# Zeng-Yan/centermask2

Measured on AMD Instinct MI355X. Metric: images/sec whole-node (V2-39-eSE 3x800x1280), higher is better.
Workload: dtype f32

## Files before the change

centermask2_amd/csrc/conv_args.hpp:

```cpp
#pragma once
#include "cmk_common.hpp"

namespace cmk {

typedef float f32x16 __attribute__((ext_vector_type(16)));
typedef float f32x4 __attribute__((ext_vector_type(4)));

constexpr int PST = 20;
constexpr int MAXP = 10;
constexpr int LDS_CU = 160 * 1024;

__host__ __device__ constexpr int occ_of(int wm, int wn, int stride) { return (stride == 1 && (wm == 1 ? wn <= 5 : wn <= 2)) ? 3 : 2; }

struct ConvProblem {
    const float* x; float* y; const float* scale; const float* shift;
    const float* in_scale; const float* in_shift;
    const float* w;
    float acc_scale;
    int N, H, W, Ho, Wo;
    int tiles_h, tiles_w, tile_begin;
    long total_pix;
};

struct ConvArgs {
// ... 7 lines not shown
    int total_tiles;
    int ksplit;
    float* ws;
    double* gn_ws;
    int gn_cpg, gn_groups;
    int ga_stride;
    float* pool_ws;
    int grid_y;
};

struct DeviceOnce {
    unsigned char done[64] = {0};
    template <typename F>
    int run(F&& f) {
        int dev = 0;
        if (hipGetDevice(&dev) != hipSuccess || dev < 0 || dev >= 64) return fail(CMK_ELAUNCH, "hipGetDevice failed%s", "");
        if (__atomic_load_n(&done[dev], __ATOMIC_ACQUIRE)) return CMK_OK;
        int rc = f();
        if (rc == CMK_OK) __atomic_store_n(&done[dev], 1, __ATOMIC_RELEASE);
        return rc;
    }
};

int launch_wino6(ConvArgs& a, int geo, hipStream_t st);
int launch_wino6s(ConvArgs& a, int geo, hipStream_t st);
int launch_pw(ConvArgs& a, int mt, hipStream_t st);
int launch_pw_split(ConvArgs& a, int mode, hipStream_t st);
int launch_sp3(ConvArgs& a, int geo, int pieces, hipStream_t st);

}
```

centermask2_amd/csrc/conv_igemm.hip:

```cpp
#include <stdlib.h>

#include "conv_args.hpp"

namespace cmk {

template <int TAPS, int STRIDE, int WM, int WN, int SC>
struct Geo {
    static constexpr int SR = 32 / SC;
    static constexpr int SUBT = 4 * WM;
    static constexpr int BM = 32 * SUBT;
    static constexpr int BN = 32 * WN;
    static constexpr int TH = (TAPS == 9) ? SR * SUBT : 1;
    static constexpr int TW = (TAPS == 9) ? SC : BM;
    static constexpr int HH = (TAPS == 9) ? (TH - 1) * STRIDE + 3 : 1;
    static constexpr int HWD = (TAPS == 9) ? (TW - 1) * STRIDE + 3 : BM;
    static constexpr int APIX = HH * HWD;
    static constexpr int A_BYTES = APIX * PST * 4;
    static constexpr int B_BYTES = BN * PST * 4;
    static constexpr int OCC = occ_of(WM, WN, STRIDE);
    static constexpr bool ADB = (2 * A_BYTES + 2 * B_BYTES) * OCC <= LDS_CU;
    static constexpr int LDS_BYTES = (ADB ? 2 : 1) * A_BYTES + 2 * B_BYTES;
    static constexpr int RESIDENT = (LDS_BYTES * OCC <= LDS_CU) ? OCC : (LDS_BYTES * 2 <= LDS_CU ? 2 : 1);
    static constexpr int A_ITERS = (APIX * 4 + 255) / 256;
    static constexpr int B_ITERS = (BN * 4 + 255) / 256;
// ... 853 lines not shown

static int dispatch(ConvArgs& a, const cmk_conv_desc* d, const cmk_conv_desc* descs, int n, hipStream_t st) {
    const int cout32 = (d->Cout + 31) / 32;
    if (d->gn_ws) {
        if (d->tune_wm != 5 && d->tune_wm != 6 && d->tune_wm != 11)
            return fail(CMK_EINVAL, "conv: fused GroupNorm statistics are only produced by the Winograd form%s", "");
        int rc = setup_gn(a, d);
        if (rc) return rc;
    }
    if (d->tune_wm == 5) {
        if (d->ksize != 3 || d->stride != 1 || d->res_mode != 0 || d->in_relu || !d->w_wino)
            return fail(CMK_EINVAL, "conv: Winograd variant not available for this conv%s", "");
        if (d->splitk > 1) return fail(CMK_EINVAL, "conv: split-K is a direct-kernel feature%s", "");
        a.w = d->w_wino;
        return launch_wino(a, st);
    }
    if (d->tune_wm == 6) {
        if (d->ksize != 3 || d->stride != 1 || d->res_mode != 0 || d->in_relu || !d->w_wino6 || (d->Cin & 7))
            return fail(CMK_EINVAL, "conv: Winograd F(4x4,3x3) variant not available for this conv%s", "");
        a.w = d->w_wino6;
        a.ws = d->splitk_ws;
        a.ksplit = d->splitk > 1 ? d->splitk : 1;
        a.cout_pad = cmk_conv_cout_pad(d->Cout);
        if (a.ksplit > 1) {
            if (d->tune_sc == 64 || d->tune_wn != 1 || n != 1) return fail(CMK_EINVAL, "conv: Winograd split-K needs tune_sc 16, tune_wn 1, one problem%s", "");
            return launch_wino6(a, 0, st);
        }
        if (d->tune_wn != 1 && d->tune_wn != 2) return fail(CMK_EINVAL, "conv: tune_wm 6 takes tune_wn 1 (12x40 map tiles) or 2 (pairs of RoI maps up to 16x14)%s", "");
        if (d->tune_sc == 64) return launch_wino6s(a, d->tune_wn == 2 ? 1 : 0, st);
        return launch_wino6(a, d->tune_wn == 2 ? 1 : 0, st);
    }
    a.ksplit = d->splitk > 1 ? d->splitk : 1;
    a.ws = d->splitk_ws;
    if (d->pool_ws && !pointwise_mt(d, n)) return fail(CMK_EINVAL, "conv: pooled sums are produced by the pointwise GEMM kernel only (cmk_conv_pool_rows)%s", "");
    a.pool_ws = d->pool_ws;
    if (d->tune_wm == 8) {
        if (d->ksize != 1 || cout32 <= 7) return fail(CMK_EINVAL, "conv: pointwise variant needs a 1x1 conv with Cout > 224%s", "");
        a.cout_pad = cdiv(cout32, 4) * 128;
        if (a.ksplit > 1 && !pointwise_mt(d, n)) return fail(CMK_EINVAL, "conv: pointwise variant: split-K not available for this conv%s", "");
        return launch_pw(a, d->tune_wn, st);
    }
    if (d->tune_wm == 10) {
        if (!(d->ksize == 1 ? pointwise_mt(d, n) : gather_mt(d, n)))
            return fail(CMK_EINVAL, "conv: the bf16-split variant needs w_split and a conv the pointwise GEMM kernel takes (1x1, or 3x3 in its gather form)%s", "");
        a.cout_pad = cdiv(cout32, 4) * 128;
        a.w = reinterpret_cast<const float*>(d->w_split);
        a.ksplit = 1;
        a.ga_stride = d->ksize == 3 ? d->stride : 0;
        return launch_pw_split(a, 1, st);
    }
    if (d->tune_wm == 12) {
        if (!(d->ksize == 1 ? pointwise_mt(d, n) : gather_mt(d, n)) || !(d->w_splith_scale > 0.f))
            return fail(CMK_EINVAL, "conv: the fp16-split variant needs w_splith, w_splith_scale and a conv the pointwise GEMM kernel takes (1x1, or 3x3 in its gather form)%s", "");
// ... 132 lines not shown
```

centermask2_amd/csrc/conv_wino6.hip:

```cpp
#include <type_traits>

#include "wino6_common.hpp"

namespace cmk {

constexpr int W6_EX_FLOATS = 4 * 4 * 2 * 8 * 64;
template <int GEO> constexpr int w6_lds_bytes() { return (2 * W6G<GEO>::WB * 16 > W6_EX_FLOATS * 4) ? 2 * W6G<GEO>::WB * 16 : W6_EX_FLOATS * 4; }
static_assert(2 * w6_lds_bytes<0>() <= LDS_CU && 2 * w6_lds_bytes<1>() <= LDS_CU, "two workgroups per CU");

template <bool AFF, int GEO>
__global__ __launch_bounds__(256, 2) void conv_wino6_kernel(const ConvArgs a) {
    using G = W6G<GEO>;
    constexpr int W6_AP = G::AP, W6_WB = G::WB;
    extern __shared__ __attribute__((aligned(16))) float smem[];
    f32x4* sW = reinterpret_cast<f32x4*>(smem);

    const int tid = threadIdx.x;
    const int lane = tid & 63;
    const int wave = __builtin_amdgcn_readfirstlane(tid >> 6);
    const int hh = lane >> 5, li = lane & 31;

    const int xq = blockIdx.x >> 3, xcd = blockIdx.x & 7;
    const int bx = (xq / a.grid_y) * 8 + xcd, by = xq % a.grid_y;
    if (bx >= a.total_tiles) return;
    int pi = 0;
#pragma unroll
    for (int i = 1; i < MAXP; ++i)
        if (i < a.nprob && bx >= a.p[i].tile_begin) pi = i;
    const ConvProblem& P = a.p[pi];
    const int H = P.H, W = P.W;
    const int tile = bx - P.tile_begin;
    int n, oh0, ow0;
    if (GEO == 0) {
        const int tw = tile % P.tiles_w;
        const int t2 = tile / P.tiles_w;
        const int th = t2 % P.tiles_h;
        n = t2 / P.tiles_h;
        oh0 = th * G::OH; ow0 = tw * G::OW;
    } else {
        n = tile * 2; oh0 = 0; ow0 = 0;
    }
    const int co0 = by * 32;
    const int ks = blockIdx.y;
    const int c_lo = (int)((long)ks * (a.Cin >> 3) / a.ksplit);
    const int nchunks = (int)((long)(ks + 1) * (a.Cin >> 3) / a.ksplit);

    int p_img, p_q, p_t, p_col;
    bool p_active;
    G::item_of(tid, p_img, p_q, p_t, p_col, p_active);
    i32x4 rsrc;
    {
        const int img_n = n + (GEO == 1 ? (wave >> 1) : 0);
        const unsigned long long base = (unsigned long long)(P.x + (long)min(img_n, P.N - 1) * H * W * a.x_cs);
        rsrc.x = __builtin_amdgcn_readfirstlane((int)(base & 0xffffffffull));
        rsrc.y = __builtin_amdgcn_readfirstlane((int)((base >> 32) & 0xffffull));
        rsrc.z = __builtin_amdgcn_readfirstlane(img_n < P.N ? H * W * a.x_cs * 4 : 0);
        rsrc.w = 0x00020000;
    }
    const int row_bytes = W * a.x_cs * 4;
    const int ih0 = oh0 - 1 + 4 * p_t, iw = ow0 - 1 + p_col;
    const int voff0 = (iw >= 0 && iw < W) ? (ih0 * W + iw) * a.x_cs * 4 + (a.x_co + p_q * 4) * 4 : (int)0x80000000;
    unsigned okm = 0;
    if (AFF) {
#pragma unroll
        for (int i = 0; i < 6; ++i) okm |= ((iw >= 0 && iw < W && ih0 + i >= 0 && ih0 + i < H) ? 1u : 0u) << i;
    }
    const unsigned aff_off = AFF ? (unsigned)(min(n + p_img, P.N - 1) * a.Cin + p_q * 4) : 0u;
    const f32x2 five = {5.0f, 5.0f};
    f32x4 d[6];
    f32x4 in_sc = {1.f, 1.f, 1.f, 1.f}, in_sh = {0.f, 0.f, 0.f, 0.f};
    auto load_D = [&](int chunk) {
#pragma unroll
        for (int i = 0; i < 6; ++i) d[i] = w6_buffer_load(rsrc, voff0 + i * row_bytes, chunk * 32, 0);
        if (AFF) {
            in_sc = *reinterpret_cast<const f32x4*>(P.in_scale + chunk * 8 + aff_off);
            in_sh = *reinterpret_cast<const f32x4*>(P.in_shift + chunk * 8 + aff_off);
        }
    };
    const int p_dst = w6_slot<GEO>(p_q, (GEO == 1 ? 4 * p_img : 0) + p_t, 0, p_col);
    auto pass1 = [&](f32x4* wbuf) {
        if (AFF) {
#pragma unroll
            for (int i = 0; i < 6; ++i) {
                const float kinf = ((okm >> i) & 1u) ? __builtin_inff() : 0.f;
                const f32x4 v = __builtin_elementwise_fma(d[i], in_sc, in_sh);
                d[i] = f32x4{__builtin_amdgcn_fmed3f(v.x, 0.f, kinf), __builtin_amdgcn_fmed3f(v.y, 0.f, kinf),
                             __builtin_amdgcn_fmed3f(v.z, 0.f, kinf), __builtin_amdgcn_fmed3f(v.w, 0.f, kinf)};
            }
        }
        f32x2* dst = reinterpret_cast<f32x2*>(wbuf + p_dst);
        if (GEO == 1 && !p_active) return;
#pragma unroll
        for (int h = 0; h < 2; ++h) {
            f32x2 e[6];
#pragma unroll
            for (int i = 0; i < 6; ++i) e[i] = h ? f32x2{d[i].z, d[i].w} : f32x2{d[i].x, d[i].y};
            f32x2 w0, w1, w2, w3, w4, w5;
            w6_half_first(e[0], e[1], e[2], e[3], e[4], five, w0, w1, w2);
            w6_half_second(e[1], e[2], e[3], e[4], e[5], five, w3, w4, w5);
            dst[0 * 2 * W6_AP + h] = w0; dst[1 * 2 * W6_AP + h] = w1; dst[2 * 2 * W6_AP + h] = w2;
            dst[3 * 2 * W6_AP + h] = w3; dst[4 * 2 * W6_AP + h] = w4; dst[5 * 2 * W6_AP + h] = w5;
        }
    };

    const int rowA = wave, rowB = 4 + (wave >> 1), halfB = wave & 1;
    int m_img, m_t, m_tc;
    G::tile_of(min(li, G::TILES - 1), m_img, m_t, m_tc);
    const f32x4* wl = sW + w6_slot<GEO>(hh, (GEO == 1 ? 4 * m_img : 0) + m_t, 0, 4 * m_tc);
    const f32x4* wA = wl + rowA * W6_AP;
    const f32x4* wB = wl + rowB * W6_AP;
    const f32x4* wBa = wB + (halfB ? G::CK : 0);
    const f32x4* wB3 = wB + (halfB ? 1 : 3 * G::CK);
    const float* u_wave = P.w + ((long)by * 4 + wave) * (9 * 256);
    const long u_chunk = (long)a.grid_y * (36 * 256);
    const int u_lane_off = lane * 4;
    f32x4 ub[3][3];
    auto load_U = [&](int step, int buf) {
        const int c = step / 3, s = step - c * 3;
        const float* src = u_wave + c * u_chunk + s * (3 * 256);
#pragma unroll
        for (int k = 0; k < 3; ++k) ub[buf][k] = *reinterpret_cast<const f32x4*>(src + (u_lane_off + k * 256));
    };
    const int total_steps = nchunks * 3;

    if (GEO == 1) {
        for (int i = tid; i < 2 * 2 * G::RG * 6 * 3; i += 256) {
            const int c3 = i % 3, rest = i / 3;
            const int a6 = rest % 6, r2 = rest / 6;
            const int r = r2 % G::RG, qb = r2 / G::RG;
            sW[(qb >> 1) * G::WB + w6_slot<GEO>(qb & 1, r, a6, 15 + c3)] = f32x4{0.f, 0.f, 0.f, 0.f};
        }
    }
    load_D(c_lo);
    f32x4 d_first[6];
#pragma unroll
    for (int i = 0; i < 6; ++i) d_first[i] = d[i];
    f32x4 sc_first = in_sc, sh_first = in_sh;
    load_D(min(c_lo + 1, nchunks - 1));
    load_U(c_lo * 3, 0);
    load_U(min(c_lo * 3 + 1, total_steps - 1), 1);
    {
        f32x4 d_keep[6], sc_keep = in_sc, sh_keep = in_sh;
#pragma unroll
        for (int i = 0; i < 6; ++i) { d_keep[i] = d[i]; d[i] = d_first[i]; }
        in_sc = sc_first; in_sh = sh_first;
        pass1(sW);
#pragma unroll
        for (int i = 0; i < 6; ++i) d[i] = d_keep[i];
        in_sc = sc_keep; in_sh = sh_keep;
    }

    f32x16 acc[9];
#pragma unroll
    for (int f = 0; f < 9; ++f)
#pragma unroll
        for (int r = 0; r < 16; ++r) acc[f][r] = 0.f;

    struct X5 { f32x2 x0, x1, x2, x3, x4; };
    auto rd = [&](const f32x4* wrow, bool second, int h) {
        const f32x2* w2 = reinterpret_cast<const f32x2*>(wrow) + h;
        X5 x;
        constexpr int K = G::CK;
        if (!second) { x.x0 = w2[0 * 2]; x.x1 = w2[K * 2]; x.x2 = w2[2 * K * 2]; x.x3 = w2[3 * K * 2]; x.x4 = w2[1 * 2]; }
        else         { x.x0 = w2[K * 2]; x.x1 = w2[2 * K * 2]; x.x2 = w2[3 * K * 2]; x.x3 = w2[1 * 2]; x.x4 = w2[(K + 1) * 2]; }
        return x;
// ... 10 lines not shown
        for (int s = 0; s < 2; ++s) {
            acc[abase + 0] = __builtin_amdgcn_mfma_f32_32x32x2f32(v0[s], ub[sbuf][0][2 * h + s], acc[abase + 0], 0, 0, 0);
            acc[abase + 1] = __builtin_amdgcn_mfma_f32_32x32x2f32(v1[s], ub[sbuf][1][2 * h + s], acc[abase + 1], 0, 0, 0);
            acc[abase + 2] = __builtin_amdgcn_mfma_f32_32x32x2f32(v2[s], ub[sbuf][2][2 * h + s], acc[abase + 2], 0, 0, 0);
        }
    };
    auto half_step = [&](const X5& x, bool second, int h, int sbuf, int abase) {
        f32x2 v0, v1, v2;
        if (!second) w6_half_first(x.x0, x.x1, x.x2, x.x3, x.x4, five, v0, v1, v2);
        else w6_half_second(x.x0, x.x1, x.x2, x.x3, x.x4, five, v0, v1, v2);
        mm(v0, v1, v2, h, sbuf, abase);
    };
    auto half_stepB = [&](const X5& x, int h) {
        f32x2 v0, v1, v2;
        if (halfB == 0) { asm volatile("" ::: "memory"); w6_half_first(x.x0, x.x1, x.x2, x.x3, x.x4, five, v0, v1, v2); }
        else            { asm volatile("" ::: "memory"); w6_half_second(x.x0, x.x1, x.x2, x.x3, x.x4, five, v0, v1, v2); }
        mm(v0, v1, v2, h, 2, 6);
    };
    auto period = [&](const int c, auto parity) {
        constexpr int wcur = decltype(parity)::value * W6_WB;
        f32x4* wnext = sW + (1 - decltype(parity)::value) * W6_WB;
        const int step = c * 3;
        __syncthreads();
        constexpr bool AHEAD = !AFF;
        load_U(min(step + 2, total_steps - 1), 2);
        X5 xa = rd(wA + wcur, false, 0), xb;
        if (AHEAD) xb = rd(wA + wcur, false, 1);
        half_step(xa, false, 0, 0, 0);
        if (AHEAD) xa = rd(wA + wcur, true, 0); else xb = rd(wA + wcur, false, 1);
        half_step(xb, false, 1, 0, 0);
        __builtin_amdgcn_sched_barrier(0);
        pass1(wnext);
        load_D(min(c + 2, nchunks - 1));
        __builtin_amdgcn_sched_barrier(0);
        load_U(min(step + 3, total_steps - 1), 0);
        if (AHEAD) xb = rd(wA + wcur, true, 1); else xa = rd(wA + wcur, true, 0);
        half_step(xa, true, 0, 1, 3);
        if (AHEAD) xa = rdB(wBa + wcur, wB3 + wcur, 0); else xb = rd(wA + wcur, true, 1);
        half_step(xb, true, 1, 1, 3);
        __builtin_amdgcn_sched_barrier(0);
        load_U(min(step + 4, total_steps - 1), 1);
        if (AHEAD) xb = rdB(wBa + wcur, wB3 + wcur, 1); else xa = rdB(wBa + wcur, wB3 + wcur, 0);
        half_stepB(xa, 0);
        if (!AHEAD) xb = rdB(wBa + wcur, wB3 + wcur, 1);
        half_stepB(xb, 1);
    };
    for (int c = c_lo; c < nchunks; c += 2) {
        period(c, std::integral_constant<int, 0>{});
        period(c + 1, std::integral_constant<int, 1>{});
    }

    const int co = co0 + li;
    const bool cvalid = co < a.Cout;
    float sc = P.scale[min(co, a.Cout - 1)];
    float sh = P.shift[min(co, a.Cout - 1)];
    __syncthreads();
    asm volatile("s_waitcnt vmcnt(0)\n\tv_mov_b32 %0, %0\n\tv_mov_b32 %1, %1" : "+v"(sc), "+v"(sh) : : "memory");
    const bool raw = a.ksplit > 1;
    float* const ybuf = raw ? a.ws + (long)ks * P.total_pix * a.cout_pad : P.y;
    const int ycs = raw ? a.cout_pad : a.y_cs, yco = raw ? 0 : a.y_co;
    if (raw) { sc = 1.f; sh = 0.f; }
    f32x2* ex2 = reinterpret_cast<f32x2*>(smem);
    const float lo = (co < a.relu_upto && !raw) ? 0.f : __builtin_nanf("");
    const f32x2 sc2 = {sc, sc}, sh2 = {sh, sh};
    auto fma2 = [](f32x2 x, float k, f32x2 y) { return __builtin_elementwise_fma(x, f32x2{k, k}, y); };
    const bool want_stats = a.gn_ws != nullptr;
    f32x2 gs2 = {0.f, 0.f}, gss2 = {0.f, 0.f};
    float gs = 0.f, gss = 0.f;
    float* yimg = ybuf + (long)n * H * W * ycs + yco + co;
    unsigned long long ybase_s;
    {
        const unsigned long long yb = (unsigned long long)(ybuf + (long)n * H * W * ycs);
        ybase_s = ((unsigned long long)(unsigned)__builtin_amdgcn_readfirstlane((int)(yb >> 32)) << 32) | (unsigned)__builtin_amdgcn_readfirstlane((int)yb);
    }
    const unsigned long long px_b = (unsigned long long)ycs * 4u, rowskip_b = (unsigned long long)(W - 3) * ycs * 4u;
#pragma unroll
    for (int q = 0; q < 2; ++q) {
        f32x2 own[8];
#pragma unroll
        for (int dd = 0; dd < 4; ++dd) {
            const int r0 = 4 * dd + 2 * q;
            f32x2 v[8];
            {
                const f32x2 m0 = {acc[0][r0], acc[0][r0 + 1]}, m1 = {acc[1][r0], acc[1][r0 + 1]}, m2 = {acc[2][r0], acc[2][r0 + 1]},
                            m3 = {acc[3][r0], acc[3][r0 + 1]}, m4 = {acc[4][r0], acc[4][r0 + 1]}, m5 = {acc[5][r0], acc[5][r0 + 1]};
// ... 97 lines not shown
#pragma unroll
                for (int j = 0; j < 4; ++j) {
                    const f32x2 t = yv[i][j] * mask;
                    gs2 += t;
                    gss2 = __builtin_elementwise_fma(t, yv[i][j], gss2);
                }
        }
        if (q == 0) __syncthreads();
    }
    gs += gs2.x + gs2.y;
    gss += gss2.x + gss2.y;
    if (a.gn_ws) {
        for (int o = 1; o < a.gn_cpg; o <<= 1) { gs += __shfl_xor(gs, o); gss += __shfl_xor(gss, o); }
        gs += __shfl_xor(gs, 32);
        gss += __shfl_xor(gss, 32);
        if (cvalid && hh == 0 && (li & (a.gn_cpg - 1)) == 0) {
            double* o = a.gn_ws + (((long)bx * 4 + wave) * a.gn_groups + co / a.gn_cpg) * 2;
            o[0] = (double)gs;
            o[1] = (double)gss;
        }
    }
}

template <int GEO>
static int launch_wino6_geo(ConvArgs& a, hipStream_t st) {
    static DeviceOnce once;
    int rc = once.run([]() {
        hipError_t e = hipFuncSetAttribute(reinterpret_cast<const void*>(conv_wino6_kernel<false, GEO>), hipFuncAttributeMaxDynamicSharedMemorySize, w6_lds_bytes<GEO>());
        if (e == hipSuccess)
            e = hipFuncSetAttribute(reinterpret_cast<const void*>(conv_wino6_kernel<true, GEO>), hipFuncAttributeMaxDynamicSharedMemorySize, w6_lds_bytes<GEO>());
        return e == hipSuccess ? CMK_OK : fail(CMK_ELAUNCH, "conv_wino6: hipFuncSetAttribute failed: %s", hipGetErrorString(e));
    });
    if (rc) return rc;
    int blocks = 0;
    for (int i = 0; i < a.nprob; ++i) {
        ConvProblem& p = a.p[i];
        p.tile_begin = blocks;
        if (GEO == 0) {
            p.tiles_h = cdiv(p.Ho, W6G<0>::OH);
            p.tiles_w = cdiv(p.Wo, W6G<0>::OW);
            blocks += p.N * p.tiles_h * p.tiles_w;
        } else {
            p.tiles_h = p.tiles_w = 1;
            blocks += cdiv(p.N, 2);
        }
    }
    a.grid_y = cdiv(a.Cout, 32);
    a.total_tiles = blocks;
    if (a.ksplit < 1) a.ksplit = 1;
    const dim3 grid(((blocks + 7) / 8) * 8 * a.grid_y, a.ksplit);
    if (a.p[0].in_scale)
        hipLaunchKernelGGL((conv_wino6_kernel<true, GEO>), grid, dim3(256), w6_lds_bytes<GEO>(), st, a);
    else
        hipLaunchKernelGGL((conv_wino6_kernel<false, GEO>), grid, dim3(256), w6_lds_bytes<GEO>(), st, a);
    return check_launch("conv_wino6");
}

int launch_wino6(ConvArgs& a, int geo, hipStream_t st) {
    for (int i = 0; i < a.nprob; ++i)
        if ((long)(geo == 0 ? 1 : 2) * a.p[i].H * a.p[i].W * std::max(a.y_cs, a.cout_pad) * 4 >= (1L << 32))
            return fail(CMK_EINVAL, "conv_wino6: an output image of 4 GiB or more%s", "");
    if (a.ksplit > 1 && (a.nprob != 1 || a.gn_ws || !a.ws || ((a.Cin >> 3) % (2 * a.ksplit)) || a.cout_pad < cdiv(a.Cout, 32) * 32))
        return fail(CMK_EINVAL, "conv_wino6: split-K takes one problem, no GroupNorm statistics, a workspace and Cin / 8 chunks %% (2 * splitk) == 0%s", "");
    if (geo == 0) return launch_wino6_geo<0>(a, st);
    if (a.nprob != 1 || a.p[0].H > 16 || a.p[0].W > 14 || a.gn_ws)
        return fail(CMK_EINVAL, "conv_wino6: the RoI-pair geometry takes one problem of maps up to 16x14 and produces no GroupNorm statistics%s", "");
    return launch_wino6_geo<1>(a, st);
}

}

extern "C" int64_t cmk_wino6_packed_floats(int Cout, int Cin) {
    return (int64_t)((Cin + 7) / 8) * ((Cout + 31) / 32) * 36 * 256;
}
```

centermask2_amd/csrc/conv_wino6s.hip:

```cpp
#include <type_traits>

#include "wino6_common.hpp"

namespace cmk {

__device__ f32x2 w6s_buffer_load2(i32x4 rsrc, int voffset, int soffset, int aux) __asm("llvm.amdgcn.raw.buffer.load.v2f32");

template <int GEO> struct W6S {
    using G = W6G<GEO>;
    static constexpr int V_SLOTS = 36 * 64;
    static constexpr int W_OFF = 2 * V_SLOTS;
    static constexpr int SLOTS = 2 * V_SLOTS + 2 * G::WB;
    static constexpr int EX_BYTES = 2 * 64 * 1024;
    static constexpr int LDS_BYTES = SLOTS * 16 > EX_BYTES ? SLOTS * 16 : EX_BYTES;
    static constexpr int ITEMS = GEO == 0 ? 3 * G::HC * 4 : 4 * G::HC * 4;
    __device__ static __forceinline__ void item_of(int tid, int& img, int& q, int& pair, int& t, int& col, bool& active) {
        const int i = GEO == 0 ? tid : (tid & 255);
        img = GEO == 0 ? 0 : (tid >> 8);
        active = i < ITEMS;
        const int j = min(i, ITEMS - 1);
        pair = j & 1; q = (j >> 1) & 1;
        const int cc = j >> 2;
        t = cc / G::HC; col = cc - t * G::HC;
    }
};
static_assert(W6S<0>::LDS_BYTES <= LDS_CU && W6S<1>::LDS_BYTES <= LDS_CU, "one workgroup per CU");
static_assert(W6S<0>::ITEMS <= 512 && W6S<1>::ITEMS <= 256, "one pass-1 item per thread");

template <bool AFF, int GEO>
// ... 43 lines not shown
    i32x4 rsrc;
    {
        const int img_n = n + (GEO == 1 ? (wave >> 2) : 0);
        const unsigned long long base = (unsigned long long)(P.x + (long)min(img_n, P.N - 1) * H * W * a.x_cs);
        rsrc.x = __builtin_amdgcn_readfirstlane((int)(base & 0xffffffffull));
        rsrc.y = __builtin_amdgcn_readfirstlane((int)((base >> 32) & 0xffffull));
        rsrc.z = __builtin_amdgcn_readfirstlane(img_n < P.N ? H * W * a.x_cs * 4 : 0);
        rsrc.w = 0x00020000;
    }
    const int row_bytes = W * a.x_cs * 4;
    const int ih0 = oh0 - 1 + 4 * p_t, iw = ow0 - 1 + p_col;
    const int voff0 = (iw >= 0 && iw < W) ? (ih0 * W + iw) * a.x_cs * 4 + (a.x_co + p_q * 4 + p_pair * 2) * 4 : (int)0x80000000;
    unsigned okm = 0;
    if (AFF) {
#pragma unroll
        for (int i = 0; i < 6; ++i) okm |= ((iw >= 0 && iw < W && ih0 + i >= 0 && ih0 + i < H) ? 1u : 0u) << i;
    }
    const unsigned aff_off = AFF ? (unsigned)(min(n + p_img, P.N - 1) * a.Cin + p_q * 4 + p_pair * 2) : 0u;
    const f32x2 five = {5.0f, 5.0f};
    f32x2 d[6];
    f32x2 in_sc = {1.f, 1.f}, in_sh = {0.f, 0.f};
    auto load_D = [&](int chunk) {
#pragma unroll
        for (int i = 0; i < 6; ++i) d[i] = w6s_buffer_load2(rsrc, voff0 + i * row_bytes, chunk * 32, 0);
        if (AFF) {
            in_sc = *reinterpret_cast<const f32x2*>(P.in_scale + chunk * 8 + aff_off);
            in_sh = *reinterpret_cast<const f32x2*>(P.in_shift + chunk * 8 + aff_off);
        }
    };
    const int p_dst2 = w6_slot<GEO>(p_q, (GEO == 1 ? 4 * p_img : 0) + p_t, 0, p_col) * 2 + p_pair;
    f32x2* const wwr2 = reinterpret_cast<f32x2*>(sW) + p_dst2;
    auto pass1 = [&](f32x2* dst) {
        if (AFF) {
#pragma unroll
            for (int i = 0; i < 6; ++i) {
                const float kinf = ((okm >> i) & 1u) ? __builtin_inff() : 0.f;
                const f32x2 v = __builtin_elementwise_fma(d[i], in_sc, in_sh);
                d[i] = f32x2{__builtin_amdgcn_fmed3f(v.x, 0.f, kinf), __builtin_amdgcn_fmed3f(v.y, 0.f, kinf)};
            }
        }
        if (GEO == 1 && !p_active) return;
        f32x2 w0, w1, w2, w3, w4, w5;
        w6_half_first(d[0], d[1], d[2], d[3], d[4], five, w0, w1, w2);
        w6_half_second(d[1], d[2], d[3], d[4], d[5], five, w3, w4, w5);
        dst[0 * 2 * AP] = w0; dst[1 * 2 * AP] = w1; dst[2 * 2 * AP] = w2;
        dst[3 * 2 * AP] = w3; dst[4 * 2 * AP] = w4; dst[5 * 2 * AP] = w5;
    };
// ... 383 lines not shown
```

centermask2_amd/csrc/wino6_common.hpp:

```cpp
#pragma once
#include "conv_args.hpp"

namespace cmk {

typedef float f32x2 __attribute__((ext_vector_type(2)));
typedef int i32x4 __attribute__((ext_vector_type(4)));

__device__ f32x4 w6_buffer_load(i32x4 rsrc, int voffset, int soffset, int aux) __asm("llvm.amdgcn.raw.buffer.load.v4f32");

template <int GEO> struct W6G;
template <> struct W6G<0> {
    static constexpr int OH = 12, OW = 40, HC = 42, CK = 12, AP = 48, TP = 6 * 48 + 10, RG = 3, QP = RG * TP, WB = 2 * QP;
    static constexpr int ITEMS = 3 * HC * 2;
    static constexpr int TILES = 30;
    __device__ static __forceinline__ void tile_of(int m, int& img, int& t, int& tc) { img = 0; t = (m * 205) >> 11; tc = m - t * 10; }
    __device__ static __forceinline__ void item_of(int tid, int& img, int& q, int& t, int& col, bool& active) {
        const int i = min(tid, ITEMS - 1);
        img = 0; q = i & 1; const int cc = i >> 1; t = cc / HC; col = cc - t * HC; active = true;
    }
};
template <> struct W6G<1> {
    static constexpr int OH = 16, OW = 14, HC = 15, CK = 5, AP = 20, TP = 6 * 20 + 12, RG = 8, QP = RG * TP, WB = 2 * QP;
    static constexpr int ITEMS = 256;
    static constexpr int TILES = 32;
    __device__ static __forceinline__ void tile_of(int m, int& img, int& t, int& tc) { img = m >> 4; t = (m >> 2) & 3; tc = m & 3; }
    __device__ static __forceinline__ void item_of(int tid, int& img, int& q, int& t, int& col, bool& active) {
        img = tid >> 7; const int i = tid & 127; active = i < 4 * HC * 2;
        const int j = min(i, 4 * HC * 2 - 1); q = j & 1; const int cc = j >> 1; t = cc / HC; col = cc - t * HC;
    }
};
static_assert(W6G<0>::TP % 16 == 10 && W6G<1>::TP % 16 == 4, "conflict-free W image");
// ... 36 lines not shown
```

centermask2_amd/ops.py:

```python
import ctypes
import os
from typing import List, Optional, Sequence, Tuple

import torch

from . import _lib
from ._lib import ConvDesc, FcosLevel, check


def _stream() -> ctypes.c_void_p:
    return ctypes.c_void_p(torch.cuda.current_stream().cuda_stream)


def _need_gpu(t: torch.Tensor, what: str) -> None:
    if not t.is_cuda:
        raise _lib.CmkError("{}: tensor is on {}; the CenterMask2 HIP path needs a GPU (no CPU fallback)".format(what, t.device))
    if t.dtype != torch.float32:
        raise _lib.CmkError("{}: expected float32, got {}".format(what, t.dtype))
    _need_current_device(t, what)


def _need_current_device(t: torch.Tensor, what: str) -> None:
    cur = torch.cuda.current_device()
    if t.device.index is not None and t.device.index != cur:
# ... 228 lines not shown

def _str_to_key(s: str):
    head, shapes = s.rsplit("_", 1)
    f = head.split("_")
    k, stride = f[0][1:].split("s")
    vals = [int(f[1][3:]), int(f[2][4:]), int(f[3][3:]), int(f[4][3:]), int(f[5][3:])]
    return (int(k), int(stride), vals[0], vals[1], vals[2], vals[3], vals[4], tuple(tuple(int(v) for v in t.split("x")) for t in shapes.split("+")))


def save_tuned(path: str) -> None:
    import json
    with open(path, "w") as f:
        json.dump({_key_to_str(k): list(v) for k, v in sorted(_TUNED.items(), key=lambda kv: _key_to_str(kv[0]))}, f, indent=0)


def _variant4(tv) -> tuple:
    return tuple(tv[:3]) + (tv[3] if len(tv) > 3 else 1,)


def _variant_on_menu(tv) -> bool:
    wm, sc, wn, sk = _variant4(tv)
    if wm == 6 and sc == 64:
        return wn in (1, 2) and sk == 1
    if wm == 10:
        return ALLOW_SPLIT_BF16 and sc == 32 and wn == 4 and sk == 1
    if wm == 12:
        return ALLOW_SPLIT_F16 and sc == 32 and wn == 4 and sk == 1
    if wm == 11:
        return ALLOW_SPLIT_F16 and sc in (2, 21) and 0 <= wn <= 3 and sk == 1
    return (wm in (1, 2, 5, 6, 7, 8, 9) and sc in (16, 32) and 1 <= wn <= 7 and sk in (1, 2, 4, 8)) or (wm, sc, wn) == (0, 0, 0)


def load_tuned(path: str) -> int:
    import json
    with open(path) as f:
        table = json.load(f)
    n = 0
    for k, v in table.items():
        if _variant_on_menu(v):
            _TUNED[_str_to_key(k)] = tuple(v)
            n += 1
    return n


def _out_pixels(d) -> int:
    ho = d.H if d.stride == 1 else (d.H - 1) // 2 + 1
# ... 27 lines not shown
    small = n == 1 and d0.res_mode != 2 and _out_pixels(d0) <= 32768
    sks = (1, 2, 4, 8) if small else (1,)
    cands = [(wm, sc, wn, sk) for wn in range(1, 8) for wm in (1, 2) for sc in (16, 32) for sk in sks]
    if small and d0.ksize == 3:
        cands += [(7, 32, wn, sk) for wn in (1, 2, 4) for sk in sks]
    if d0.ksize == 3:
        cands += [(9, 32, mt, sk) for mt in (4, 2) for sk in sks]
        if ALLOW_SPLIT_BF16:
            cands += [(10, 32, 4, 1)]
        if ALLOW_SPLIT_F16:
            cands += [(12, 32, 4, 1)]
            cands += [(11, 2, g, 1) for g in range(4)]
            cands += [(11, 21, g, 1) for g in range(4)]
    if d0.ksize == 1:
        cands += [(8, 32, mt, sk) for mt in (4, 2) for sk in sks]
        if ALLOW_SPLIT_BF16:
            cands += [(10, 32, 4, 1)]
        if ALLOW_SPLIT_F16:
            cands += [(12, 32, 4, 1)]
    if ALLOW_WINOGRAD:
        cands += [(5, 16, 2, 1)]
        cands += [(6, 16, 1, 1), (6, 16, 2, 1)]
        cands += [(6, 64, 1, 1), (6, 64, 2, 1)]
        if small and d0.ksize == 3:
            cands += [(6, 16, 1, sk) for sk in (2, 4)]
    if TUNE_ONLY is not None:
        cands = [_variant4(tv) for tv in TUNE_ONLY(key)]
    times = {}
    for _ in range(TUNE_ROUNDS):
        for tv in cands:
            if times.get(tv) == float("inf"):
                continue
            ws = _set_variant(descs, n, tv)
            if run() != 0:
                times[tv] = float("inf")
                continue
            e0, e1 = torch.cuda.Event(enable_timing=True), torch.cuda.Event(enable_timing=True)
            e0.record()
            for _r in range(TUNE_REPS):
                run()
            e1.record()
            e1.synchronize()
            times[tv] = min(times.get(tv, float("inf")), e0.elapsed_time(e1) / TUNE_REPS)
            del ws
    for tv in cands:
        if times.get(tv, float("inf")) < best_ms:
            best, best_ms = (tv[:3] if tv[3] == 1 else tv), times[tv]
    _TUNED[key] = best
# ... 432 lines not shown
    return out


PROFILE = None


def kernel_source_hash() -> str:
    import hashlib
    import os
    h = hashlib.sha1()
    d = os.path.join(os.path.dirname(os.path.abspath(__file__)), "csrc")
    for f in ("conv_args.hpp", "wino6_common.hpp", "conv_igemm.hip", "conv_wino6.hip", "conv_wino6s.hip", "conv_pw.hip", "conv_sp3.hip"):
        h.update(open(os.path.join(d, f), "rb").read())
    return h.hexdigest()[:12]


def executed_flops(taps: int, stride: int, tv, shapes, cin_pad: int, cout: int) -> float:
    cd = lambda a, b: -(-a // b)
    wm, sc, wn = (tuple(tv[:3]) if tv else (0, 0, 0))
    if wm == 5:
        return float(sum(n * cd(h, 8) * cd(w, 16) for n, h, w in shapes) * cd(cout, 64) * (cin_pad // 16) * 256 * 4096)
    if wm == 6:
        wgs = sum(cd(n, 2) for n, h, w in shapes) if wn == 2 else sum(n * cd(h, 12) * cd(w, 40) for n, h, w in shapes)
        return float(wgs * cd(cout, 32) * (cin_pad // 8) * 144 * 4096)
    if wm == 11:
        th, tw, ct = ((8, 32, 128), (4, 32, 256), (16, 16, 128), (8, 16, 256))[wn]
        if sc == 21 or (wn == 0 and cout <= 64):
            ct //= 2
        return float(sum(n * cd(h, th) * cd(w, tw) for n, h, w in shapes) * th * tw) * (cd(cout, ct) * ct) * cin_pad * 9 * 2.0
    cout_pad = _lib.load().cmk_conv_cout_pad(cout)
    if wm in (8, 9, 10, 12):
        return float(sum(cd(n * h * w, 64 * wn) for n, h, w in shapes)) * (64 * wn) * (cd(cout, 128) * 128) * cin_pad * taps * 2.0
    if wm not in (1, 2):
        wm, sc = 1, (32 if taps == 1 else 16)
    if taps == 9 and tuple(tv[:1]) != (7,):
        thh, tww = (32 // sc) * 4 * wm, sc
        tiles = sum(n * cd(h, thh) * cd(w, tww) for n, h, w in shapes)
    else:
        tiles = sum(cd(n * h * w, 128 * wm) for n, h, w in shapes)
    return float(tiles) * (128 * wm) * cout_pad * taps * cin_pad * 2.0


def _kernel_name(taps, stride, tv, aff=False, pool=False, upres=False, cout=None) -> str:
    if tv[0] == 5:
        return "conv_wino4r_kernel<{}>".format("true" if aff else "false")
    if tv[0] == 6:
        return "conv_wino6{}_kernel<{}, {}>".format("s" if tv[1] == 64 else "", "true" if aff else "false", 1 if tv[2] == 2 else 0)
    wm, sc, wn = tv[:3]
    sk = "true" if (len(tv) > 3 and tv[3] > 1) else "false"
    if wm == 8:
        return "conv_pw_kernel<{}, {}, false, {}, {}, 0>".format(wn, "true" if pool else "false", "true" if upres else "false", sk)
    if wm in (10, 12):
        return "conv_pw_kernel<4, {}, {}, {}, false, {}>".format("true" if pool else "false", "true" if taps == 9 else "false", "true" if upres else "false", 1 if wm == 10 else 2)
    if wm == 11:
        return "conv_sp3_kernel<{}, {}, 2, {}>".format(wn, 1 if (sc == 21 or (wn == 0 and cout is not None and cout <= 64)) else 2, "true" if aff else "false")
    if wm == 9:
        return "conv_pw_kernel<{}, false, true, false, {}, 0>".format(wn, sk)
    if wm == 7:
        return "conv_igemm_kernel<1, 1, 1, {}, 32, true>".format(wn)
    return "conv_igemm_kernel<{}, {}, {}, {}, {}, false>".format(taps, stride, wm, wn, 32 if taps == 1 else sc)


def preprocess_images(images: Sequence[torch.Tensor], mean, std, size_divisibility: int = 32, fixed_size: Optional[int] = None):
    lib = _lib.load()
    sizes = [(int(im.shape[-2]), int(im.shape[-1])) for im in images]
    if fixed_size:
        H = W = int(fixed_size)
    else:
        d = max(1, size_divisibility)
        H = (max(s[0] for s in sizes) + d - 1) // d * d
# ... 23 lines not shown
```

Before: 365.2.

## Add paired 512-thread Winograd F(4x4,3x3) variant covering two cout tiles

Adds a paired form of the Winograd-6 conv kernel in which one 512-thread workgroup computes two 32-channel output tiles. The input-transform work is split across the thread pairs, each handling two channels, so the transformed input tile in LDS is built once and shared by both cout halves instead of being recomputed by separate workgroups. The variant is exposed as tune_sc 32 and added to the autotuner candidates, with doubled epilogue exchange space in LDS. The costs are one workgroup per CU, more LDS per workgroup, and a clamp on the second cout tile when the channel-tile count is odd.

```diff
diff --git a/centermask2_amd/csrc/conv_args.hpp b/centermask2_amd/csrc/conv_args.hpp
--- a/centermask2_amd/csrc/conv_args.hpp
+++ b/centermask2_amd/csrc/conv_args.hpp
@@ -53,7 +53,7 @@
     }
 };
 
-int launch_wino6(ConvArgs& a, int geo, hipStream_t st);
+int launch_wino6(ConvArgs& a, int geo, bool pair, hipStream_t st);
 int launch_wino6s(ConvArgs& a, int geo, hipStream_t st);
 int launch_pw(ConvArgs& a, int mt, hipStream_t st);
 int launch_pw_split(ConvArgs& a, int mode, hipStream_t st);
diff --git a/centermask2_amd/csrc/conv_igemm.hip b/centermask2_amd/csrc/conv_igemm.hip
--- a/centermask2_amd/csrc/conv_igemm.hip
+++ b/centermask2_amd/csrc/conv_igemm.hip
@@ -899,13 +899,16 @@
         a.ws = d->splitk_ws;
         a.ksplit = d->splitk > 1 ? d->splitk : 1;
         a.cout_pad = cmk_conv_cout_pad(d->Cout);
+        if (d->tune_sc != 0 && d->tune_sc != 16 && d->tune_sc != 32 && d->tune_sc != 64)
+            return fail(CMK_EINVAL, "conv: tune_wm 6 takes tune_sc 16 (32 couts per workgroup), 32 (paired) or 64 (shared V)%s", "");
+        const bool pair = d->tune_sc == 32;
         if (a.ksplit > 1) {
-            if (d->tune_sc == 64 || d->tune_wn != 1 || n != 1) return fail(CMK_EINVAL, "conv: Winograd split-K needs tune_sc 16, tune_wn 1, one problem%s", "");
-            return launch_wino6(a, 0, st);
+            if (d->tune_sc == 64 || d->tune_wn != 1 || n != 1) return fail(CMK_EINVAL, "conv: Winograd split-K needs tune_sc 16 or 32, tune_wn 1, one problem%s", "");
+            return launch_wino6(a, 0, pair, st);
         }
         if (d->tune_wn != 1 && d->tune_wn != 2) return fail(CMK_EINVAL, "conv: tune_wm 6 takes tune_wn 1 (12x40 map tiles) or 2 (pairs of RoI maps up to 16x14)%s", "");
         if (d->tune_sc == 64) return launch_wino6s(a, d->tune_wn == 2 ? 1 : 0, st);
-        return launch_wino6(a, d->tune_wn == 2 ? 1 : 0, st);
+        return launch_wino6(a, d->tune_wn == 2 ? 1 : 0, pair, st);
     }
     a.ksplit = d->splitk > 1 ? d->splitk : 1;
     a.ws = d->splitk_ws;
diff --git a/centermask2_amd/csrc/conv_wino6.hip b/centermask2_amd/csrc/conv_wino6.hip
--- a/centermask2_amd/csrc/conv_wino6.hip
+++ b/centermask2_amd/csrc/conv_wino6.hip
@@ -5,23 +5,32 @@
 namespace cmk {
 
 constexpr int W6_EX_FLOATS = 4 * 4 * 2 * 8 * 64;
-template <int GEO> constexpr int w6_lds_bytes() { return (2 * W6G<GEO>::WB * 16 > W6_EX_FLOATS * 4) ? 2 * W6G<GEO>::WB * 16 : W6_EX_FLOATS * 4; }
+template <int GEO, bool PAIR = false> constexpr int w6_lds_bytes() {
+    return (2 * W6G<GEO>::WB * 16 > (PAIR ? 2 : 1) * W6_EX_FLOATS * 4) ? 2 * W6G<GEO>::WB * 16 : (PAIR ? 2 : 1) * W6_EX_FLOATS * 4;
+}
 static_assert(2 * w6_lds_bytes<0>() <= LDS_CU && 2 * w6_lds_bytes<1>() <= LDS_CU, "two workgroups per CU");
-
-template <bool AFF, int GEO>
-__global__ __launch_bounds__(256, 2) void conv_wino6_kernel(const ConvArgs a) {
+static_assert(w6_lds_bytes<0, true>() <= LDS_CU && w6_lds_bytes<1, true>() <= LDS_CU, "paired form: one workgroup per CU");
+
+template <bool AFF, int GEO, bool PAIR>
+__device__ __forceinline__ void conv_wino6_body(const ConvArgs& a) {
     using G = W6G<GEO>;
     constexpr int W6_AP = G::AP, W6_WB = G::WB;
+    constexpr int NT = PAIR ? 512 : 256;
     extern __shared__ __attribute__((aligned(16))) float smem[];
     f32x4* sW = reinterpret_cast<f32x4*>(smem);
 
     const int tid = threadIdx.x;
     const int lane = tid & 63;
-    const int wave = __builtin_amdgcn_readfirstlane(tid >> 6);
+    const int wid = __builtin_amdgcn_readfirstlane(tid >> 6);
+    const int wave = PAIR ? (wid & 3) : wid;
+    const int half = PAIR ? (wid >> 2) : 0;
     const int hh = lane >> 5, li = lane & 31;
 
+    const int gy = PAIR ? (a.grid_y + 1) >> 1 : a.grid_y;
     const int xq = blockIdx.x >> 3, xcd = blockIdx.x & 7;
-    const int bx = (xq / a.grid_y) * 8 + xcd, by = xq % a.grid_y;
+    const int bx = (xq / gy) * 8 + xcd, by = xq % gy;
+    const int ctile = PAIR ? 2 * by + half : by;
+    const int ct = PAIR ? min(ctile, a.grid_y - 1) : by;
     if (bx >= a.total_tiles) return;
     int pi = 0;
 #pragma unroll
@@ -40,17 +49,18 @@
     } else {
         n = tile * 2; oh0 = 0; ow0 = 0;
     }
-    const int co0 = by * 32;
+    const int co0 = ctile * 32;
     const int ks = blockIdx.y;
     const int c_lo = (int)((long)ks * (a.Cin >> 3) / a.ksplit);
     const int nchunks = (int)((long)(ks + 1) * (a.Cin >> 3) / a.ksplit);
 
     int p_img, p_q, p_t, p_col;
     bool p_active;
-    G::item_of(tid, p_img, p_q, p_t, p_col, p_active);
+    G::item_of(PAIR ? (tid >> 1) : tid, p_img, p_q, p_t, p_col, p_active);
+    const int p_h = PAIR ? (tid & 1) : 0;
     i32x4 rsrc;
     {
-        const int img_n = n + (GEO == 1 ? (wave >> 1) : 0);
+        const int img_n = n + (GEO == 1 ? (PAIR ? (wid >> 2) : (wave >> 1)) : 0);
         const unsigned long long base = (unsigned long long)(P.x + (long)min(img_n, P.N - 1) * H * W * a.x_cs);
         rsrc.x = __builtin_amdgcn_readfirstlane((int)(base & 0xffffffffull));
         rsrc.y = __builtin_amdgcn_readfirstlane((int)((base >> 32) & 0xffffull));
@@ -59,22 +69,28 @@
     }
     const int row_bytes = W * a.x_cs * 4;
     const int ih0 = oh0 - 1 + 4 * p_t, iw = ow0 - 1 + p_col;
-    const int voff0 = (iw >= 0 && iw < W) ? (ih0 * W + iw) * a.x_cs * 4 + (a.x_co + p_q * 4) * 4 : (int)0x80000000;
+    const int voff0 = (iw >= 0 && iw < W) ? (ih0 * W + iw) * a.x_cs * 4 + (a.x_co + p_q * 4 + p_h * 2) * 4 : (int)0x80000000;
     unsigned okm = 0;
     if (AFF) {
 #pragma unroll
         for (int i = 0; i < 6; ++i) okm |= ((iw >= 0 && iw < W && ih0 + i >= 0 && ih0 + i < H) ? 1u : 0u) << i;
     }
-    const unsigned aff_off = AFF ? (unsigned)(min(n + p_img, P.N - 1) * a.Cin + p_q * 4) : 0u;
+    const unsigned aff_off = AFF ? (unsigned)(min(n + p_img, P.N - 1) * a.Cin + p_q * 4 + p_h * 2) : 0u;
     const f32x2 five = {5.0f, 5.0f};
-    f32x4 d[6];
-    f32x4 in_sc = {1.f, 1.f, 1.f, 1.f}, in_sh = {0.f, 0.f, 0.f, 0.f};
+    using DV = std::conditional_t<PAIR, f32x2, f32x4>;
+    DV d[6];
+    DV in_sc, in_sh;
+    if constexpr (PAIR) { in_sc = f32x2{1.f, 1.f}; in_sh = f32x2{0.f, 0.f}; }
+    else { in_sc = f32x4{1.f, 1.f, 1.f, 1.f}; in_sh = f32x4{0.f, 0.f, 0.f, 0.f}; }
     auto load_D = [&](int chunk) {
 #pragma unroll
-        for (int i = 0; i < 6; ++i) d[i] = w6_buffer_load(rsrc, voff0 + i * row_bytes, chunk * 32, 0);
+        for (int i = 0; i < 6; ++i) {
+            if constexpr (PAIR) d[i] = w6_buffer_load2(rsrc, voff0 + i * row_bytes, chunk * 32, 0);
+            else d[i] = w6_buffer_load(rsrc, voff0 + i * row_bytes, chunk * 32, 0);
+        }
         if (AFF) {
-            in_sc = *reinterpret_cast<const f32x4*>(P.in_scale + chunk * 8 + aff_off);
-            in_sh = *reinterpret_cast<const f32x4*>(P.in_shift + chunk * 8 + aff_off);
+            in_sc = *reinterpret_cast<const DV*>(P.in_scale + chunk * 8 + aff_off);
+            in_sh = *reinterpret_cast<const DV*>(P.in_shift + chunk * 8 + aff_off);
         }
     };
     const int p_dst = w6_slot<GEO>(p_q, (GEO == 1 ? 4 * p_img : 0) + p_t, 0, p_col);
@@ -83,18 +99,22 @@
 #pragma unroll
             for (int i = 0; i < 6; ++i) {
                 const float kinf = ((okm >> i) & 1u) ? __builtin_inff() : 0.f;
-                const f32x4 v = __builtin_elementwise_fma(d[i], in_sc, in_sh);
-                d[i] = f32x4{__builtin_amdgcn_fmed3f(v.x, 0.f, kinf), __builtin_amdgcn_fmed3f(v.y, 0.f, kinf),
-                             __builtin_amdgcn_fmed3f(v.z, 0.f, kinf), __builtin_amdgcn_fmed3f(v.w, 0.f, kinf)};
-            }
-        }
-        f32x2* dst = reinterpret_cast<f32x2*>(wbuf + p_dst);
+                const DV v = __builtin_elementwise_fma(d[i], in_sc, in_sh);
+                if constexpr (PAIR) d[i] = f32x2{__builtin_amdgcn_fmed3f(v.x, 0.f, kinf), __builtin_amdgcn_fmed3f(v.y, 0.f, kinf)};
+                else d[i] = f32x4{__builtin_amdgcn_fmed3f(v.x, 0.f, kinf), __builtin_amdgcn_fmed3f(v.y, 0.f, kinf),
+                                  __builtin_amdgcn_fmed3f(v.z, 0.f, kinf), __builtin_amdgcn_fmed3f(v.w, 0.f, kinf)};
+            }
+        }
+        f32x2* dst = reinterpret_cast<f32x2*>(wbuf + p_dst) + p_h;
         if (GEO == 1 && !p_active) return;
 #pragma unroll
-        for (int h = 0; h < 2; ++h) {
+        for (int h = 0; h < (PAIR ? 1 : 2); ++h) {
             f32x2 e[6];
 #pragma unroll
-            for (int i = 0; i < 6; ++i) e[i] = h ? f32x2{d[i].z, d[i].w} : f32x2{d[i].x, d[i].y};
+            for (int i = 0; i < 6; ++i) {
+                if constexpr (PAIR) e[i] = d[i];
+                else e[i] = h ? f32x2{d[i].z, d[i].w} : f32x2{d[i].x, d[i].y};
+            }
             f32x2 w0, w1, w2, w3, w4, w5;
             w6_half_first(e[0], e[1], e[2], e[3], e[4], five, w0, w1, w2);
             w6_half_second(e[1], e[2], e[3], e[4], e[5], five, w3, w4, w5);
@@ -111,7 +131,7 @@
     const f32x4* wB = wl + rowB * W6_AP;
     const f32x4* wBa = wB + (halfB ? G::CK : 0);
     const f32x4* wB3 = wB + (halfB ? 1 : 3 * G::CK);
-    const float* u_wave = P.w + ((long)by * 4 + wave) * (9 * 256);
+    const float* u_wave = P.w + ((long)ct * 4 + wave) * (9 * 256);
     const long u_chunk = (long)a.grid_y * (36 * 256);
     const int u_lane_off = lane * 4;
     f32x4 ub[3][3];
@@ -124,7 +144,7 @@
     const int total_steps = nchunks * 3;
 
     if (GEO == 1) {
-        for (int i = tid; i < 2 * 2 * G::RG * 6 * 3; i += 256) {
+        for (int i = tid; i < 2 * 2 * G::RG * 6 * 3; i += NT) {
             const int c3 = i % 3, rest = i / 3;
             const int a6 = rest % 6, r2 = rest / 6;
             const int r = r2 % G::RG, qb = r2 / G::RG;
@@ -132,15 +152,15 @@
         }
     }
     load_D(c_lo);
-    f32x4 d_first[6];
+    DV d_first[6];
 #pragma unroll
     for (int i = 0; i < 6; ++i) d_first[i] = d[i];
-    f32x4 sc_first = in_sc, sh_first = in_sh;
+    DV sc_first = in_sc, sh_first = in_sh;
     load_D(min(c_lo + 1, nchunks - 1));
     load_U(c_lo * 3, 0);
     load_U(min(c_lo * 3 + 1, total_steps - 1), 1);
     {
-        f32x4 d_keep[6], sc_keep = in_sc, sh_keep = in_sh;
+        DV d_keep[6], sc_keep = in_sc, sh_keep = in_sh;
 #pragma unroll
         for (int i = 0; i < 6; ++i) { d_keep[i] = d[i]; d[i] = d_first[i]; }
         in_sc = sc_first; in_sh = sh_first;
@@ -197,7 +217,7 @@
         f32x4* wnext = sW + (1 - decltype(parity)::value) * W6_WB;
         const int step = c * 3;
         __syncthreads();
-        constexpr bool AHEAD = !AFF;
+        constexpr bool AHEAD = !AFF || PAIR;
         load_U(min(step + 2, total_steps - 1), 2);
         X5 xa = rd(wA + wcur, false, 0), xb;
         if (AHEAD) xb = rd(wA + wcur, false, 1);
@@ -235,7 +255,7 @@
     float* const ybuf = raw ? a.ws + (long)ks * P.total_pix * a.cout_pad : P.y;
     const int ycs = raw ? a.cout_pad : a.y_cs, yco = raw ? 0 : a.y_co;
     if (raw) { sc = 1.f; sh = 0.f; }
-    f32x2* ex2 = reinterpret_cast<f32x2*>(smem);
+    f32x2* ex2 = reinterpret_cast<f32x2*>(smem + half * W6_EX_FLOATS);
     const float lo = (co < a.relu_upto && !raw) ? 0.f : __builtin_nanf("");
     const f32x2 sc2 = {sc, sc}, sh2 = {sh, sh};
     auto fma2 = [](f32x2 x, float k, f32x2 y) { return __builtin_elementwise_fma(x, f32x2{k, k}, y); };
@@ -379,13 +399,26 @@
     }
 }
 
-template <int GEO>
+template <bool AFF, int GEO>
+__global__ __launch_bounds__(256, 2) void conv_wino6_kernel(const ConvArgs a) {
+    conv_wino6_body<AFF, GEO, false>(a);
+}
+
+template <bool AFF, int GEO>
+__global__ __launch_bounds__(512, 2) void conv_wino6p_kernel(const ConvArgs a) {
+    conv_wino6_body<AFF, GEO, true>(a);
+}
+
+template <int GEO, bool PAIR>
 static int launch_wino6_geo(ConvArgs& a, hipStream_t st) {
     static DeviceOnce once;
-    int rc = once.run([]() {
-        hipError_t e = hipFuncSetAttribute(reinterpret_cast<const void*>(conv_wino6_kernel<false, GEO>), hipFuncAttributeMaxDynamicSharedMemorySize, w6_lds_bytes<GEO>());
+    const auto k_plain = PAIR ? conv_wino6p_kernel<false, GEO> : conv_wino6_kernel<false, GEO>;
+    const auto k_aff = PAIR ? conv_wino6p_kernel<true, GEO> : conv_wino6_kernel<true, GEO>;
+    constexpr int lds = w6_lds_bytes<GEO, PAIR>();
+    int rc = once.run([&]() {
+        hipError_t e = hipFuncSetAttribute(reinterpret_cast<const void*>(k_plain), hipFuncAttributeMaxDynamicSharedMemorySize, lds);
         if (e == hipSuccess)
-            e = hipFuncSetAttribute(reinterpret_cast<const void*>(conv_wino6_kernel<true, GEO>), hipFuncAttributeMaxDynamicSharedMemorySize, w6_lds_bytes<GEO>());
+            e = hipFuncSetAttribute(reinterpret_cast<const void*>(k_aff), hipFuncAttributeMaxDynamicSharedMemorySize, lds);
         return e == hipSuccess ? CMK_OK : fail(CMK_ELAUNCH, "conv_wino6: hipFuncSetAttribute failed: %s", hipGetErrorString(e));
     });
     if (rc) return rc;
@@ -405,24 +438,27 @@
     a.grid_y = cdiv(a.Cout, 32);
     a.total_tiles = blocks;
     if (a.ksplit < 1) a.ksplit = 1;
-    const dim3 grid(((blocks + 7) / 8) * 8 * a.grid_y, a.ksplit);
-    if (a.p[0].in_scale)
-        hipLaunchKernelGGL((conv_wino6_kernel<true, GEO>), grid, dim3(256), w6_lds_bytes<GEO>(), st, a);
-    else
-        hipLaunchKernelGGL((conv_wino6_kernel<false, GEO>), grid, dim3(256), w6_lds_bytes<GEO>(), st, a);
-    return check_launch("conv_wino6");
-}
-
-int launch_wino6(ConvArgs& a, int geo, hipStream_t st) {
+    const dim3 grid(((blocks + 7) / 8) * 8 * (PAIR ? cdiv(a.grid_y, 2) : a.grid_y), a.ksplit);
+    if constexpr (PAIR) {
+        if (a.p[0].in_scale) hipLaunchKernelGGL((conv_wino6p_kernel<true, GEO>), grid, dim3(512), lds, st, a);
+        else hipLaunchKernelGGL((conv_wino6p_kernel<false, GEO>), grid, dim3(512), lds, st, a);
+    } else {
+        if (a.p[0].in_scale) hipLaunchKernelGGL((conv_wino6_kernel<true, GEO>), grid, dim3(256), lds, st, a);
+        else hipLaunchKernelGGL((conv_wino6_kernel<false, GEO>), grid, dim3(256), lds, st, a);
+    }
+    return check_launch(PAIR ? "conv_wino6p" : "conv_wino6");
+}
+
+int launch_wino6(ConvArgs& a, int geo, bool pair, hipStream_t st) {
     for (int i = 0; i < a.nprob; ++i)
         if ((long)(geo == 0 ? 1 : 2) * a.p[i].H * a.p[i].W * std::max(a.y_cs, a.cout_pad) * 4 >= (1L << 32))
             return fail(CMK_EINVAL, "conv_wino6: an output image of 4 GiB or more%s", "");
     if (a.ksplit > 1 && (a.nprob != 1 || a.gn_ws || !a.ws || ((a.Cin >> 3) % (2 * a.ksplit)) || a.cout_pad < cdiv(a.Cout, 32) * 32))
         return fail(CMK_EINVAL, "conv_wino6: split-K takes one problem, no GroupNorm statistics, a workspace and Cin / 8 chunks %% (2 * splitk) == 0%s", "");
-    if (geo == 0) return launch_wino6_geo<0>(a, st);
+    if (geo == 0) return pair ? launch_wino6_geo<0, true>(a, st) : launch_wino6_geo<0, false>(a, st);
     if (a.nprob != 1 || a.p[0].H > 16 || a.p[0].W > 14 || a.gn_ws)
         return fail(CMK_EINVAL, "conv_wino6: the RoI-pair geometry takes one problem of maps up to 16x14 and produces no GroupNorm statistics%s", "");
-    return launch_wino6_geo<1>(a, st);
+    return pair ? launch_wino6_geo<1, true>(a, st) : launch_wino6_geo<1, false>(a, st);
 }
 
 }
diff --git a/centermask2_amd/csrc/conv_wino6s.hip b/centermask2_amd/csrc/conv_wino6s.hip
--- a/centermask2_amd/csrc/conv_wino6s.hip
+++ b/centermask2_amd/csrc/conv_wino6s.hip
@@ -3,8 +3,6 @@
 #include "wino6_common.hpp"
 
 namespace cmk {
-
-__device__ f32x2 w6s_buffer_load2(i32x4 rsrc, int voffset, int soffset, int aux) __asm("llvm.amdgcn.raw.buffer.load.v2f32");
 
 template <int GEO> struct W6S {
     using G = W6G<GEO>;
@@ -94,7 +92,7 @@
     f32x2 in_sc = {1.f, 1.f}, in_sh = {0.f, 0.f};
     auto load_D = [&](int chunk) {
 #pragma unroll
-        for (int i = 0; i < 6; ++i) d[i] = w6s_buffer_load2(rsrc, voff0 + i * row_bytes, chunk * 32, 0);
+        for (int i = 0; i < 6; ++i) d[i] = w6_buffer_load2(rsrc, voff0 + i * row_bytes, chunk * 32, 0);
         if (AFF) {
             in_sc = *reinterpret_cast<const f32x2*>(P.in_scale + chunk * 8 + aff_off);
             in_sh = *reinterpret_cast<const f32x2*>(P.in_shift + chunk * 8 + aff_off);
diff --git a/centermask2_amd/csrc/wino6_common.hpp b/centermask2_amd/csrc/wino6_common.hpp
--- a/centermask2_amd/csrc/wino6_common.hpp
+++ b/centermask2_amd/csrc/wino6_common.hpp
@@ -7,6 +7,7 @@
 typedef int i32x4 __attribute__((ext_vector_type(4)));
 
 __device__ f32x4 w6_buffer_load(i32x4 rsrc, int voffset, int soffset, int aux) __asm("llvm.amdgcn.raw.buffer.load.v4f32");
+__device__ f32x2 w6_buffer_load2(i32x4 rsrc, int voffset, int soffset, int aux) __asm("llvm.amdgcn.raw.buffer.load.v2f32");
 
 template <int GEO> struct W6G;
 template <> struct W6G<0> {
diff --git a/centermask2_amd/ops.py b/centermask2_amd/ops.py
--- a/centermask2_amd/ops.py
+++ b/centermask2_amd/ops.py
@@ -274,6 +274,8 @@
     wm, sc, wn, sk = _variant4(tv)
     if wm == 6 and sc == 64:
         return wn in (1, 2) and sk == 1
+    if wm == 6:
+        return sc in (16, 32) and wn in (1, 2) and sk in (1, 2, 4, 8)
     if wm == 10:
         return ALLOW_SPLIT_BF16 and sc == 32 and wn == 4 and sk == 1
     if wm == 12:
@@ -347,8 +349,9 @@
         cands += [(5, 16, 2, 1)]
         cands += [(6, 16, 1, 1), (6, 16, 2, 1)]
         cands += [(6, 64, 1, 1), (6, 64, 2, 1)]
+        cands += [(6, 32, 1, 1), (6, 32, 2, 1)]
         if small and d0.ksize == 3:
-            cands += [(6, 16, 1, sk) for sk in (2, 4)]
+            cands += [(6, sc, 1, sk) for sc in (16, 32) for sk in (2, 4)]
     if TUNE_ONLY is not None:
         cands = [_variant4(tv) for tv in TUNE_ONLY(key)]
     times = {}
@@ -827,7 +830,7 @@
         return float(sum(n * cd(h, 8) * cd(w, 16) for n, h, w in shapes) * cd(cout, 64) * (cin_pad // 16) * 256 * 4096)
     if wm == 6:
         wgs = sum(cd(n, 2) for n, h, w in shapes) if wn == 2 else sum(n * cd(h, 12) * cd(w, 40) for n, h, w in shapes)
-        return float(wgs * cd(cout, 32) * (cin_pad // 8) * 144 * 4096)
+        return float(wgs * (2 * cd(cout, 64) if sc == 32 else cd(cout, 32)) * (cin_pad // 8) * 144 * 4096)
     if wm == 11:
         th, tw, ct = ((8, 32, 128), (4, 32, 256), (16, 16, 128), (8, 16, 256))[wn]
         if sc == 21 or (wn == 0 and cout <= 64):
@@ -850,7 +853,7 @@
     if tv[0] == 5:
         return "conv_wino4r_kernel<{}>".format("true" if aff else "false")
     if tv[0] == 6:
-        return "conv_wino6{}_kernel<{}, {}>".format("s" if tv[1] == 64 else "", "true" if aff else "false", 1 if tv[2] == 2 else 0)
+        return "conv_wino6{}_kernel<{}, {}>".format({64: "s", 32: "p"}.get(tv[1], ""), "true" if aff else "false", 1 if tv[2] == 2 else 0)
     wm, sc, wn = tv[:3]
     sk = "true" if (len(tv) > 3 and tv[3] > 1) else "false"
     if wm == 8:
```

Result: faster. 374.1, median of 6 (+2.4%).
